# antonilo/unsupervised_detection

Measured on NVIDIA H100. Metric: frame-pairs/sec adversarial train step 256x448, higher is better.
Workload: dtype bf16

## Files before the change

### include/cis_b200.h

```cpp
#ifndef CIS_B200_H_
#define CIS_B200_H_
#include <stdint.h>
#include <stddef.h>

#ifdef __cplusplus
extern "C" {
#endif

typedef void* cis_stream_t;

enum { CIS_OK = 0, CIS_ERR_BAD_ARG = 1, CIS_ERR_UNSUPPORTED = 2, CIS_ERR_CUDA = 3 };
enum { CIS_ACT_NONE = 0, CIS_ACT_ELU = 1, CIS_ACT_LEAKY = 2 };
enum { CIS_MAX_TAPS = 49, CIS_MAX_SRC = 4 };

typedef struct {
  const void* ptr;
  int32_t pitch;
  int32_t c_off;
  int32_t chunks;
  int32_t n_mod;
} CisSrc;

typedef struct {
  int32_t N, H, W;
// ... 52 lines not shown
  int16_t dw[CIS_MAX_TAPS];
  int32_t nsrc;
  CisSrc src[CIS_MAX_SRC];
  const void* g;
  int32_t g_pitch, g_coff, g_chunks;
  float* dwp;
  int32_t Cout;
  int32_t K_pad;
  int32_t splits;
  int32_t tma;
  int32_t nh;
  int32_t nwg;
} CisWgrad;

const char* cis_last_error(void);
int cis_version(void);
uint32_t cis_crc32c(uint32_t crc, const void* data, size_t n);
int cis_host_resize_bilinear_legacy(const float* src, int32_t H, int32_t W, int32_t C, float* dst, int32_t OH, int32_t OW);
int cis_host_bgr8_to_rgb_resized(const unsigned char* bgr, int32_t H, int32_t W, float* dst, int32_t OH, int32_t OW);

int cis_conv_igemm(const CisConv* d, cis_stream_t stream);
int cis_conv_s2_phase_plan(const CisConv* d, CisConv* h, int16_t* wk);
int cis_set_persist_mode(int mode);
int cis_conv_wgrad(const CisWgrad* d, cis_stream_t stream);

int cis_pack_weights(const float* w, const int32_t* kmap, int32_t K_pad, int32_t rows, int32_t cout, int32_t sn, const int32_t* nmap,
                     void* wp, cis_stream_t stream);
int cis_pack_weights_tiled(const float* w, const int32_t* kmap, int32_t cin8, int32_t ntaps, int32_t n_tiles, int32_t BN, int32_t cout,
                           int32_t sn, const int32_t* nmap, void* out, int32_t thin, cis_stream_t stream);
int cis_unpack_wgrad(const float* dwp, const int32_t* kmap, int32_t K_pad, int32_t cout, int32_t nsplit, float* dw, const float* colpart,
                     int32_t nblocks, int32_t nch, float* db, int32_t layout, cis_stream_t stream);
int cis_bn_fold(const float* w, const float* bias, const float* gamma, const float* beta, int64_t nw, int32_t cout, float* w_eff,
                float* b_eff, cis_stream_t stream);
int cis_bn_chain(const float* w, const float* bias, const float* gamma, float* dw_eff_to_dw, const float* db_eff, int64_t nw,
                 int32_t cout, float* dbias, float* dgamma, float* dbeta, cis_stream_t stream);

enum { CIS_JOB_PACK = 0, CIS_JOB_PACK_TILED = 1, CIS_JOB_UNPACK = 2, CIS_JOB_BN_FOLD = 3, CIS_JOB_BN_CHAIN = 4 };
typedef struct {
  int32_t kind;
  int32_t i[8];
  int64_t n;
  const void* p[8];
} CisParamJob;
int cis_param_multi(const CisParamJob* jobs_dev, int32_t njobs, int32_t total_blocks, cis_stream_t stream);

int cis_dact_mul(void* g, int32_t g_pitch, int32_t g_coff, const void* y, int32_t y_pitch, int32_t y_coff, const void* res,
                 int32_t res_pitch, int32_t res_coff, int64_t npix, int32_t chunks, int32_t act, float alpha, cis_stream_t stream);
// ... 114 lines not shown
```

### unsupervised_detection_b200/_lib.py

```python
import ctypes as C
import os

_HERE = os.path.dirname(os.path.abspath(__file__))
LIB_PATH = os.path.join(_HERE, os.environ.get('CIS_LIB_NAME', 'libcis_b200.so'))

MAX_TAPS, MAX_SRC = 49, 4
ACT_NONE, ACT_ELU, ACT_LEAKY = 0, 1, 2
RESIZE_BILINEAR, RESIZE_NEAREST = 0, 1


class CisSrc(C.Structure):
    _fields_ = [('ptr', C.c_void_p), ('pitch', C.c_int32), ('c_off', C.c_int32), ('chunks', C.c_int32), ('n_mod', C.c_int32)]


class CisParamJob(C.Structure):
    _fields_ = [('kind', C.c_int32), ('i', C.c_int32 * 8), ('n', C.c_int64), ('p', C.c_void_p * 8)]


JOB_PACK, JOB_PACK_TILED, JOB_UNPACK, JOB_BN_FOLD, JOB_BN_CHAIN = range(5)


class CisSub(C.Structure):
    _fields_ = [('tap0', C.c_int32), ('ntaps', C.c_int32), ('hoy', C.c_int32), ('hox', C.c_int32), ('OH', C.c_int32), ('OW', C.c_int32),
                ('oa', C.c_int32), ('ob', C.c_int32), ('wpack', C.c_void_p)]
# ... 8 lines not shown
                ('bias', C.c_void_p), ('act', C.c_int32), ('alpha', C.c_float),
                ('DH', C.c_int32), ('DW', C.c_int32), ('osh', C.c_int32), ('osw', C.c_int32), ('oa', C.c_int32), ('ob', C.c_int32),
                ('out', C.c_void_p), ('out_pitch', C.c_int32), ('out_coff', C.c_int32), ('out_ch', C.c_int32),
                ('outf', C.c_void_p), ('outf_pitch', C.c_int32), ('outf_coff', C.c_int32), ('outf_ch', C.c_int32),
                ('add_pre', C.c_void_p), ('add_pre_pitch', C.c_int32), ('add_pre_coff', C.c_int32),
                ('addf_pre', C.c_void_p), ('addf_pitch', C.c_int32), ('addf_coff', C.c_int32),
                ('add_post', C.c_void_p), ('add_post_pitch', C.c_int32), ('add_post_coff', C.c_int32),
                ('mode', C.c_int32),
                ('halo', C.c_int32), ('dil', C.c_int32), ('MT', C.c_int32), ('hoy', C.c_int32), ('hox', C.c_int32),
                ('ey', C.c_int32), ('ex', C.c_int32),
                ('splits', C.c_int32), ('sk_scratch', C.c_void_p), ('sk_counters', C.c_void_p),
                ('nph', C.c_int32), ('ph_tap', C.c_int32 * 5), ('sk_cluster', C.c_int32),
                ('nsub', C.c_int32), ('sub', CisSub * 4), ('nwg', C.c_int32), ('thin', C.c_int32)]


class CisWgrad(C.Structure):
    _fields_ = [('N', C.c_int32), ('H', C.c_int32), ('W', C.c_int32), ('OH', C.c_int32), ('OW', C.c_int32),
                ('sh', C.c_int32), ('sw', C.c_int32), ('ntaps', C.c_int32),
                ('dh', C.c_int16 * MAX_TAPS), ('dw', C.c_int16 * MAX_TAPS),
                ('nsrc', C.c_int32), ('src', CisSrc * MAX_SRC),
                ('g', C.c_void_p), ('g_pitch', C.c_int32), ('g_coff', C.c_int32), ('g_chunks', C.c_int32),
                ('dwp', C.c_void_p), ('Cout', C.c_int32), ('K_pad', C.c_int32), ('splits', C.c_int32), ('tma', C.c_int32),
                ('nh', C.c_int32), ('nwg', C.c_int32)]


_i32, _i64, _f32, _p, _u64 = C.c_int32, C.c_int64, C.c_float, C.c_void_p, C.c_uint64

_PROTOS = {
    'cis_conv_igemm': [C.POINTER(CisConv)],
    'cis_conv_wgrad': [C.POINTER(CisWgrad)],
    'cis_pack_weights': [_p, _p, _i32, _i32, _i32, _i32, _p, _p],
    'cis_pack_weights_tiled': [_p, _p, _i32, _i32, _i32, _i32, _i32, _i32, _p, _p, _i32],
    'cis_unpack_wgrad': [_p, _p, _i32, _i32, _i32, _p, _p, _i32, _i32, _p, _i32],
    'cis_bn_fold': [_p, _p, _p, _p, _i64, _i32, _p, _p],
    'cis_param_multi': [_p, _i32, _i32],
    'cis_bn_chain': [_p, _p, _p, _p, _p, _i64, _i32, _p, _p, _p],
    'cis_dact_mul': [_p, _i32, _i32, _p, _i32, _i32, _p, _i32, _i32, _i64, _i32, _i32, _f32],
    'cis_add_slice': [_p, _i32, _i32, _p, _i32, _i32, _i64, _i32, _i32, _i32],
    'cis_colsum': [_p, _i32, _i32, _i64, _i32, _p, _i32],
    'cis_zero': [_p, _i64],
    'cis_dact_colsum': [_p, _i32, _i32, _p, _i32, _i32, _p, _i32, _i32, _i64, _i32, _i32, _f32, _p, _i32],
    'cis_resize_bilinear_bf16': [_p, _i32, _i32, _i32, _i32, _i32, _p, _i32, _i32, _i32, _i32, _i32],
    'cis_resize_concat_bf16': [C.POINTER(CisSrc), _i32, _i32, _i32, _i32, _p, _i32, _i32, _i32, _i32],
    'cis_resize_concat_bf16_bwd': [_p, _i32, _i32, _i32, _i32, _i32, C.POINTER(CisSrc), C.POINTER(C.c_int32), C.POINTER(C.c_int32), _i32, _i32, _i32],
    'cis_resize_bilinear_bf16_bwd': [_p, _i32, _i32, _i32, _i32, _i32, _p, _i32, _i32, _i32, _i32, _i32, _i32],
    'cis_resize_bilinear_f32': [_p, _i32, _i32, _i32, _i32, _p, _i32, _i32, _f32],
# ... 19 lines not shown
    'cis_cis_loss_reduce': [_p, _i32, _i32, _i64, _f32, _p, _p],
    'cis_cis_loss_bwd': [_p, _p, _p, _p, _p, _i32, _i32, _i32, _i32, _i32, _f32, _i32, _p, _p],
    'cis_resize_f32_bwd_to_bf16': [_p, _i32, _i32, _i32, _i32, _i32, _i32, _p, _i32],
    'cis_mask_bwd': [_p, _p, _p, _p, _i32, _i64, _p],
    'cis_abs_sum': [_p, _i64, _p],
    'cis_grad_avg_abs': [_p, _p, _i32, _p],
    'cis_clip_adam': [_p, _p, _p, _p, _i64, _f32, _f32, _f32, _f32, _f32, _f32, _p, _p, _i32, _u64],
    'cis_cast_f32_to_bf16': [_p, _i64, _p],
    'cis_cast_bf16_to_f32': [_p, _i64, _i32, _i32, _i32, _p],
    'cis_cast_bf16_to_f32_scaled': [_p, _i64, _i32, _i32, _i32, _f32, _p],
    'cis_charbonnier_bwd': [_p, _p, _p, _i32, _i64, _i32, _i32, _f32, _p, _p, _p, _p],
    'cis_dense_image_warp_bwd': [_p, _i32, _i32, _p, _f32, _i32, _i32, _i32, _i32, _p, _p, _p, _p],
    'cis_cost_volume_bwd': [_p, _i32, _i32, _p, _i32, _i32, _p, _i32, _i32, _i32, _i32, _p, _p, _p],
    'cis_resize_f32_bwd_to_bf16_scaled': [_p, _i32, _i32, _i32, _i32, _i32, _i32, _p, _i32, _f32],
    'cis_warp_costvol_bwd': [_p, _i32, _i32, _p, _i32, _i32, _p, _f32, _i32, _i32, _i32, _i32, _p, _i32, _i32, _p, _i32, _i32, _p, _i32, _i32,
                             _p, _i32, _i32, _i32, _p, _p, _p],
    'cis_parity_split_bf16': [_p, _i32, _i32, _i32, _i32, _i32, _i32, _p, _i32],
    'cis_warp_costvol_r': [_p, _i32, _i32, _p, _i32, _i32, _p, _f32, _i32, _i32, _i32, _i32, _p, _i32, _i32, _i32],
    'cis_cost_volume_bwd_r': [_p, _i32, _i32, _p, _i32, _i32, _p, _i32, _i32, _i32, _i32, _p, _p, _p, _i32],
    'cis_warp_costvol_bwd_r': [_p, _i32, _i32, _p, _i32, _i32, _p, _f32, _i32, _i32, _i32, _i32, _p, _i32, _i32, _p, _i32, _i32, _p, _i32, _i32,
                               _p, _i32, _i32, _i32, _p, _p, _p, _i32],
}
EXPORTS = sorted(list(_PROTOS) + ['cis_last_error', 'cis_version', 'cis_set_persist_mode', 'cis_crc32c', 'cis_host_resize_bilinear_legacy',
                                  'cis_host_bgr8_to_rgb_resized', 'cis_conv_s2_phase_plan'])

_lib = None


def load():
    global _lib
    if _lib is None:
        if not os.path.exists(LIB_PATH):
            raise RuntimeError('libcis_b200.so not built: run `python -c "import __graft_entry__ as g; g.build()"` '
                               '(no CPU fallback exists for the product path)')
        lib = C.CDLL(LIB_PATH)
        lib.cis_last_error.restype = C.c_char_p
        lib.cis_version.restype = C.c_int
        lib.cis_set_persist_mode.argtypes = [C.c_int]
        lib.cis_set_persist_mode.restype = C.c_int
        lib.cis_crc32c.argtypes = [C.c_uint32, C.c_void_p, C.c_size_t]
        lib.cis_crc32c.restype = C.c_uint32
        lib.cis_host_resize_bilinear_legacy.argtypes = [C.c_void_p, C.c_int32, C.c_int32, C.c_int32, C.c_void_p, C.c_int32, C.c_int32]
        lib.cis_host_resize_bilinear_legacy.restype = C.c_int
        lib.cis_host_bgr8_to_rgb_resized.argtypes = [C.c_void_p, C.c_int32, C.c_int32, C.c_void_p, C.c_int32, C.c_int32]
        lib.cis_host_bgr8_to_rgb_resized.restype = C.c_int
        lib.cis_conv_s2_phase_plan.argtypes = [C.POINTER(CisConv), C.POINTER(CisConv), C.POINTER(C.c_int16)]
        lib.cis_conv_s2_phase_plan.restype = C.c_int
        for name, args in _PROTOS.items():
            fn = getattr(lib, name)
            fn.argtypes = list(args) + [C.c_void_p]
            fn.restype = C.c_int
        _lib = lib
    return _lib


def check(rc, what=''):
    if rc != 0:
        raise RuntimeError('libcis_b200 %s failed (code %d): %s' % (what, rc, load().cis_last_error().decode()))


def call(name, *args):
    check(getattr(load(), name)(*args), name)
```

### unsupervised_detection_b200/csrc/conv_igemm.cu

```cuda
#include "ptx.cuh"
#include "../../include/cis_b200.h"
#include "common.cuh"
#include <cuda.h>
#include <stdlib.h>
#include <string.h>


namespace cis {

#ifdef CIS_TRACE
__device__ unsigned long long* g_trace = nullptr;
__device__ int g_trace_cap = 0;
#define CIS_TRACE_AT(slot)                                                                                         \
  do {                                                                                                             \
    if (g_trace && blockIdx.x == 0 && blockIdx.y == 0 && blockIdx.z == 0 && (slot) < g_trace_cap) g_trace[(slot)] = clock64(); \
  } while (0)
#else
#define CIS_TRACE_AT(slot) ((void)0)
#endif

static constexpr int kBM = 128;
static constexpr int kBK = 64;
static constexpr int kAStage = kBM * 128;
static constexpr int kThreads = 256;
// ... 1373 lines not shown
  static constexpr uint32_t kLayout = NH == 64 ? 1u : NH == 32 ? 2u : 3u;
};

template <int NH, int NWG>
__device__ __forceinline__ void wgrad_halo_wg_pairs(int w, int npairs, int cout, int& qa, int& np, int& hf) {
  constexpr int P = WgradHaloCfg<NH>::kPairs;
  const int nhalf = cout > 64 ? 2 : 1;
  if (NWG == 2 && nhalf == 2) {
    qa = blockIdx.z * P;
    np = min(P, npairs - qa);
    hf = w;
    return;
  }
  const int q0 = (blockIdx.z / nhalf) * (NWG * P);
  const int cnt = min(NWG * P, npairs - q0);
  const int h = NWG == 2 ? (cnt + 1) / 2 : cnt;
  qa = q0 + (w ? h : 0);
  np = w ? cnt - h : h;
  hf = blockIdx.z % nhalf;
}

template <int NH, int NWG>
__global__ void __launch_bounds__(128 * (1 + NWG)) conv_wgrad_halo_kernel(const __grid_constant__ CisWgrad p, const __grid_constant__ WgradHaloMaps maps,
                                                                          const int Wh, const int Hh, const int hoy, const int hox,
                                                                          const int stage_bytes, const int S) {
  using Cfg = WgradHaloCfg<NH>;
  constexpr int P = Cfg::kPairs;
  extern __shared__ uint8_t smem_raw[];
  __shared__ uint64_t bars[2 * kWHMaxStages + 1];
  __shared__ int s_off[CIS_MAX_TAPS + 1];
  const uint32_t tile_base = (smem_u32(smem_raw) + 1023u) & ~1023u;
  const uint32_t bar_full = smem_u32(&bars[0]);
  const uint32_t bar_empty = smem_u32(&bars[kWHMaxStages]);
  const uint32_t bar_accum = smem_u32(&bars[2 * kWHMaxStages]);
  const int tid = threadIdx.x, warp = tid >> 5, lane = tid & 31;
  pdl_launch_dependents();
  if (tid < p.ntaps) s_off[tid] = (p.dh[tid] - hoy) * Wh + (p.dw[tid] - hox);
  if (tid == p.ntaps) s_off[tid] = 0;
  const bool wg_halves = NWG == 2 && p.Cout > 64;
  const int ng = wg_halves ? 2 : 1;
  const int halo_bytes = stage_bytes - ng * (int)Cfg::kGTile;
  const int tiles_x = (p.OW + 7) / 8, tiles_y = (p.OH + 7) / 8;
  const int nkb_total = p.N * tiles_x * tiles_y;
  const int per = (nkb_total + (int)gridDim.y - 1) / (int)gridDim.y;
  const int kb0 = blockIdx.y * per;
  const int nkb = min(per, nkb_total - kb0);
  if (nkb <= 0) return;
  int m_chunks = 0;
  for (int i = 0; i < p.nsrc; ++i) m_chunks += p.src[i].chunks;
  const int nch64 = (m_chunks + 7) / 8;
  const int npairs = (p.ntaps + 1) / 2;
  const int c64 = blockIdx.x;

  if (tid == 128) {
    for (int s = 0; s < S; ++s) {
      mbar_init(bar_full + 8 * s, 1);
      mbar_init(bar_empty + 8 * s, NWG);
    }
    mbar_init(bar_accum, 128 * NWG);
    fence_mbar_init();
  }
// ... 1 lines not shown
  __syncthreads();

  if (warp < 4) {
    if (tid == 0) {
      int c = c64 * 8, si = 0;
      while (si < p.nsrc - 1 && c >= p.src[si].chunks) {
        c -= p.src[si].chunks;
        ++si;
      }
      int nm = p.src[0].n_mod;
      if (si == 1) nm = p.src[1].n_mod;
      if (si == 2) nm = p.src[2].n_mod;
      if (si == 3) nm = p.src[3].n_mod;
      int qa, np, hf0;
      wgrad_halo_wg_pairs<NH, NWG>(0, npairs, p.Cout, qa, np, hf0);
      const int tpi = tiles_x * tiles_y;
      for (int it = 0; it < nkb; ++it) {
        const int s = it % S;
        mbar_wait(bar_empty + 8 * s, (uint32_t)(((it / S) & 1) ^ 1));
        const int kb = kb0 + it;
        const int n = kb / tpi, r = kb - n * tpi;
        const int ty = r / tiles_x, tx = r - ty * tiles_x;
        const uint32_t st = tile_base + s * stage_bytes, bar = bar_full + 8 * s;
        mbar_expect_tx(bar, (uint32_t)(Wh * Hh * 128 + ng * (int)Cfg::kGTile));
        tma_load_4d(st, &maps.x[si], bar, c * 8, tx * 8 + hox, ty * 8 + hoy, nm ? (n % nm) : n);
        for (int h = 0; h < ng; ++h)
          tma_load_4d(st + halo_bytes + h * Cfg::kGTile, &maps.g, bar, (hf0 + h) * 64, tx * 8, ty * 8, n);
      }
    }
    __syncwarp();
    mbar_wait(bar_accum, 0);
    const int r = warp * 32 + lane;
    const int cch = r & 63;
    const uint32_t t_row = tile_base + (uint32_t)r * 16;
    for (int w = 0; w < NWG; ++w) {
      int qa, np, hf;
      wgrad_halo_wg_pairs<NH, NWG>(w, npairs, p.Cout, qa, np, hf);
      for (int q = 0; q < np; ++q) {
        const int t = 2 * (qa + q) + (r >> 6);
        if (t >= p.ntaps) continue;
        const size_t kcol = ((size_t)t * nch64 + c64) * 64 + cch;
#pragma unroll 1
        for (int c0 = 0; c0 < NH && hf * 64 + c0 < p.Cout; c0 += 16) {
          float v[16];
          acc_ld16(t_row + (uint32_t)((w * P + q) * NH + c0) * kAccColBytes, v);
          for (int e = 0; e < 16; ++e) {
            const int co = hf * 64 + c0 + e;
            if (co < p.Cout) p.dwp[((size_t)blockIdx.y * p.Cout + co) * p.K_pad + kcol] = v[e];
          }
        }
      }
    }
  } else {
    const int wg = NWG > 1 ? (warp - 4) >> 2 : 0;
    const int wtid = tid - 128 * (1 + wg);
    int qa, np, hf;
    wgrad_halo_wg_pairs<NH, NWG>(wg, npairs, p.Cout, qa, np, hf);
    np = __shfl_sync(0xffffffffu, np, 0);
    float acc[P][NH];
    const uint32_t ahi = desc_hi((uint32_t)(Wh * 128));
    const uint32_t bhi = (((8 * Cfg::kGRow) >> 4) & 0x3FFF) | (Cfg::kLayout << 30);
    const uint32_t kstep = (uint32_t)(2 * Wh * 128) >> 4;
    const uint32_t g_off = (uint32_t)halo_bytes + (wg_halves ? (uint32_t)wg * Cfg::kGTile : 0u);
    for (int it = 0; it < nkb; ++it) {
      const int s = it % S;
      mbar_wait(bar_full + 8 * s, (uint32_t)((it / S) & 1));
      const uint32_t st = tile_base + s * stage_bytes;
      const uint32_t blo0 = desc_lo(st + g_off, Cfg::kGTile);
      wg_fence();
#pragma unroll
      for (int q = 0; q < P; ++q) {
        if (q < np) {
          const int o0 = s_off[2 * (qa + q)], o1 = s_off[2 * (qa + q) + 1];
          const uint32_t lbo = (uint32_t)((o1 > o0 ? o1 - o0 : 1) * 128);
          const uint32_t alo0 = desc_lo(st + (uint32_t)(o0 * 128), lbo);
#pragma unroll
          for (int k = 0; k < 4; ++k)
            mma128<NH, 1, 1>(acc[q], alo0 + k * kstep, ahi, blo0 + Cfg::kGRow * k, bhi, lbo >> 4, (uint32_t)((it | k) != 0));
        }
      }
      wg_commit();
      wg_wait<0>();
      if (wtid == 0) mbar_arrive(bar_empty + 8 * s);
    }
    if constexpr (NWG > 1) asm volatile("bar.sync 1, %0;" ::"n"(128 * NWG) : "memory");
#pragma unroll
    for (int q = 0; q < P; ++q)
      if (q < np) acc_store<NH>(acc[q], tile_base + (uint32_t)((wg * P + q) * NH) * kAccColBytes, wtid);
    mbar_arrive(bar_accum);
  }
}

}

using namespace cis;

static bool pdl_enabled() {
  static const bool on = !(getenv("CIS_PDL") && atoi(getenv("CIS_PDL")) == 0);
  return on;
}
template <typename... KArgs, typename... Args>
static cudaError_t launch_pdl(void (*kern)(KArgs...), dim3 grid, dim3 block, size_t smem, cudaStream_t st, Args... args) {
  cudaLaunchConfig_t cfg;
  memset(&cfg, 0, sizeof(cfg));
  cfg.gridDim = grid;
  cfg.blockDim = block;
  cfg.dynamicSmemBytes = smem;
  cfg.stream = st;
  cudaLaunchAttribute attr[1];
  attr[0].id = cudaLaunchAttributeProgrammaticStreamSerialization;
  attr[0].val.programmaticStreamSerializationAllowed = 1;
// ... 377 lines not shown
      case 128: return d->nwg == 2 ? launch_halo<128, 2>(d, st) : launch_halo<128, 1>(d, st);
      default: return cis_set_error(CIS_ERR_UNSUPPORTED, "cis_conv_igemm: BN must be 16/32/64/128");
    }
  }
  CisConv h;
  int16_t wk[2 * CIS_MAX_TAPS];
  if (s2_phase_plan(d, &h, wk)) {
    switch (h.BN) {
      case 16: return launch_halo<16, 1>(&h, st, wk);
      case 32: return launch_halo<32, 1>(&h, st, wk);
      case 64: return launch_halo<64, 1>(&h, st, wk);
      case 128: return launch_halo<128, 1>(&h, st, wk);
    }
  }
  switch (d->BN) {
    case 16: return launch_fwd<16>(d, st);
    case 32: return launch_fwd<32>(d, st);
    case 64: return launch_fwd<64>(d, st);
    case 128: return launch_fwd<128>(d, st);
    default: return cis_set_error(CIS_ERR_UNSUPPORTED, "cis_conv_igemm: BN must be 16/32/64/128");
  }
}

template <int NH, int NWG>
static int launch_wgrad_halo_t(const CisWgrad* d, cudaStream_t st, int nch64, int Wh, int Hh, int hoy, int hox, int halo_bytes) {
  using Cfg = WgradHaloCfg<NH>;
  const bool wg_halves = NWG == 2 && d->Cout > 64;
  const int stage = halo_bytes + (wg_halves ? 2 : 1) * (int)Cfg::kGTile;
  const int npairs = (d->ntaps + 1) / 2, nhalf = d->Cout > 64 ? 2 : 1;
  const int gz = wg_halves ? (npairs + Cfg::kPairs - 1) / Cfg::kPairs : nhalf * ((npairs + NWG * Cfg::kPairs - 1) / (NWG * Cfg::kPairs));
  int S = (200 * 1024) / stage;
  if (S > kWHMaxStages) S = kWHMaxStages;
  if (S < 2) return cis_set_error(CIS_ERR_UNSUPPORTED, "cis_conv_wgrad(halo): halo does not fit shared memory");
  int smem = S * stage + 1024;
  const int acc_smem = NWG * kMaxAccCols * (int)kAccColBytes + 1024;
  if (smem < acc_smem) smem = acc_smem;
  static int attr_smem = 0;
  if (smem > attr_smem) {
    cudaError_t e = cudaFuncSetAttribute(conv_wgrad_halo_kernel<NH, NWG>, cudaFuncAttributeMaxDynamicSharedMemorySize, smem);
    if (e != cudaSuccess) return cis_set_cuda_error(e, "cudaFuncSetAttribute(conv_wgrad_halo)");
    attr_smem = smem;
  }
  WgradHaloMaps maps;
  memset(&maps, 0, sizeof(maps));
  CisSrc gs;
  gs.ptr = d->g; gs.pitch = d->g_pitch; gs.c_off = d->g_coff; gs.chunks = d->g_chunks; gs.n_mod = 0;
  const CUtensorMapSwizzle gswz = NH == 64 ? CU_TENSOR_MAP_SWIZZLE_128B : NH == 32 ? CU_TENSOR_MAP_SWIZZLE_64B : CU_TENSOR_MAP_SWIZZLE_32B;
  bool ok = encode_src_map(&maps.g, gs, d->N, d->OH, d->OW, 8, 8, 1, 0, 0, 1, NH, gswz);
  for (int i = 0; ok && i < d->nsrc; ++i) ok = encode_src_map(&maps.x[i], d->src[i], d->N, d->H, d->W, Wh, Hh);
  if (!ok) return cis_set_error(CIS_ERR_CUDA, "cis_conv_wgrad(halo): cuTensorMapEncodeTiled failed / unavailable");
  dim3 grid(nch64, d->splits, gz);
  cudaError_t le = launch_pdl(conv_wgrad_halo_kernel<NH, NWG>, grid, dim3(128 * (1 + NWG)), (size_t)smem, st, *d, maps, Wh, Hh, hoy, hox, stage, S);
  if (le != cudaSuccess) return cis_set_cuda_error(le, "launch(conv_wgrad_halo)");
  return cis_check_launch("conv_wgrad_halo");
}

static int launch_wgrad_halo(const CisWgrad* d, cudaStream_t st) {
  if (d->sh != 1 || d->sw != 1) return cis_set_error(CIS_ERR_BAD_ARG, "cis_conv_wgrad(halo): needs a stride-1 layer");
  int chunks = 0;
  for (int i = 0; i < d->nsrc; ++i) chunks += d->src[i].chunks;
  for (int i = 0; i < d->nsrc - 1; ++i)
    if (d->src[i].chunks % 8) return cis_set_error(CIS_ERR_BAD_ARG, "cis_conv_wgrad(halo): needs 64-channel aligned concat sources");
  const int nch64 = (chunks + 7) / 8;
  int hoy = d->dh[0], hox = d->dw[0], my = d->dh[0], mx = d->dw[0];
  for (int t = 1; t < d->ntaps; ++t) {
    if (d->dh[t] < hoy) hoy = d->dh[t];
    if (d->dw[t] < hox) hox = d->dw[t];
    if (d->dh[t] > my) my = d->dh[t];
    if (d->dw[t] > mx) mx = d->dw[t];
  }
  for (int t = 1; t < d->ntaps; ++t)
    if ((d->dh[t] - hoy) * 1024 + (d->dw[t] - hox) <= (d->dh[t - 1] - hoy) * 1024 + (d->dw[t - 1] - hox))
      return cis_set_error(CIS_ERR_BAD_ARG, "cis_conv_wgrad(halo): taps must be listed in increasing row-major order");
  const int Wh = 8 + (mx - hox), Hh = 8 + (my - hoy);
  if (Wh > 256 || Hh > 256) return cis_set_error(CIS_ERR_UNSUPPORTED, "cis_conv_wgrad(halo): tap extent too large");
  if (d->K_pad < d->ntaps * nch64 * 64) return cis_set_error(CIS_ERR_BAD_ARG, "cis_conv_wgrad(halo): K_pad smaller than taps * 64-channel groups");
  const int nh = d->nh ? d->nh : 64, nwg = d->nwg ? d->nwg : 1;
  if ((nh != 16 && nh != 32 && nh != 64) || nh < (d->Cout > 64 ? 64 : (d->Cout + 15) / 16 * 16) || nwg < 1 || nwg > 2)
    return cis_set_error(CIS_ERR_BAD_ARG, "cis_conv_wgrad(halo): nh must be 16/32/64 and cover Cout (64 above 64), nwg 1 or 2");
  const int halo_bytes = (Wh * Hh * 128 + 1023) & ~1023;
  switch (nh * 4 + nwg) {
    case 16 * 4 + 1: return launch_wgrad_halo_t<16, 1>(d, st, nch64, Wh, Hh, hoy, hox, halo_bytes);
    case 16 * 4 + 2: return launch_wgrad_halo_t<16, 2>(d, st, nch64, Wh, Hh, hoy, hox, halo_bytes);
    case 32 * 4 + 1: return launch_wgrad_halo_t<32, 1>(d, st, nch64, Wh, Hh, hoy, hox, halo_bytes);
    case 32 * 4 + 2: return launch_wgrad_halo_t<32, 2>(d, st, nch64, Wh, Hh, hoy, hox, halo_bytes);
    case 64 * 4 + 1: return launch_wgrad_halo_t<64, 1>(d, st, nch64, Wh, Hh, hoy, hox, halo_bytes);
    default: return launch_wgrad_halo_t<64, 2>(d, st, nch64, Wh, Hh, hoy, hox, halo_bytes);
  }
}

extern "C" int cis_conv_wgrad(const CisWgrad* d, cis_stream_t stream) {
  if (!d || d->ntaps < 1 || d->ntaps > CIS_MAX_TAPS || d->nsrc < 1 || d->nsrc > CIS_MAX_SRC || d->K_pad % 64 != 0 || d->Cout < 1 ||
      d->Cout > 128 || d->splits < 1 || !d->g || !d->dwp)
    return cis_set_error(CIS_ERR_BAD_ARG, "cis_conv_wgrad: bad descriptor");
  {
    const long M = (long)d->N * d->OH * d->OW;
    const long nkb_total = d->tma ? (long)d->N * ((d->OW + 7) / 8) * ((d->OH + 7) / 8) : (M + 63) / 64;
    const long per = (nkb_total + d->splits - 1) / d->splits;
    if ((long)(d->splits - 1) * per >= nkb_total) return cis_set_error(CIS_ERR_BAD_ARG, "cis_conv_wgrad: a split would own no reduction block");
  }
  if (d->tma == 2) return launch_wgrad_halo(d, (cudaStream_t)stream);
  static bool attr_set = false;
  if (!attr_set) {
    cudaError_t e = cudaFuncSetAttribute(conv_wgrad_kernel, cudaFuncAttributeMaxDynamicSharedMemorySize, kWSmem);
    if (e != cudaSuccess) return cis_set_cuda_error(e, "cudaFuncSetAttribute(conv_wgrad)");
    attr_set = true;
  }
  WgradMaps maps;
  memset(&maps, 0, sizeof(maps));
  if (d->tma) {
    if (d->sh != 1 || d->sw != 1) return cis_set_error(CIS_ERR_BAD_ARG, "cis_conv_wgrad: TMA path needs a stride-1 layer");
    for (int i = 0; i < d->nsrc - 1; ++i)
      if (d->src[i].chunks % 8) return cis_set_error(CIS_ERR_BAD_ARG, "cis_conv_wgrad: TMA path needs 64-channel aligned concat sources");
    CisSrc gs;
    gs.ptr = d->g; gs.pitch = d->g_pitch; gs.c_off = d->g_coff; gs.chunks = d->g_chunks; gs.n_mod = 0;
    bool ok = encode_src_map(&maps.g, gs, d->N, d->OH, d->OW, 8, 8);
    for (int i = 0; ok && i < d->nsrc; ++i) ok = encode_src_map(&maps.x[i], d->src[i], d->N, d->H, d->W, 8, 8);
    if (!ok) return cis_set_error(CIS_ERR_CUDA, "cis_conv_wgrad: cuTensorMapEncodeTiled failed / unavailable");
  }
  dim3 grid((d->K_pad + 127) / 128, d->splits);
  cudaError_t le = launch_pdl(conv_wgrad_kernel, grid, dim3(d->tma ? kThreads : kGThreads), kWSmem, (cudaStream_t)stream, *d, maps);
  if (le != cudaSuccess) return cis_set_cuda_error(le, "launch(conv_wgrad)");
  return cis_check_launch("conv_wgrad");
}
// ... 1 lines not shown
```

### unsupervised_detection_b200/engine.py

```python
import ctypes as C
import dataclasses
import os

import numpy as np
import torch

from . import _lib
from ._lib import CisConv, CisWgrad, CisSrc, ACT_NONE, ACT_ELU, ACT_LEAKY


def ru(x, m):
    return (x + m - 1) // m * m


def same_pad(n_in, k, s=1, d=1):
    out = -(-n_in // s)
    total = max((out - 1) * s + (k - 1) * d + 1 - n_in, 0)
    return total // 2, total - total // 2


SIDE_STREAM = True
_SIDE = {}
MULTI_PARAM_OPS = os.environ.get('CIS_MULTI_PARAM', '1') == '1'
DACT_COLSUM = os.environ.get('CIS_DACT_COLSUM', '1') == '1'
# ... 258 lines not shown
WGRAD_TMA = True
MATERIALIZE_MISALIGNED_CONCAT = True


WGRAD_CTAS_PER_SM = int(os.environ.get('CIS_WGRAD_CTAS_PER_SM', '2'))
WGRAD_MAX_SLICE_MB = float(os.environ.get('CIS_WGRAD_MAX_SLICE_MB', '16'))
WGRAD_HALO_MIN_CH = int(os.environ.get('CIS_WGRAD_HALO_MIN_CH', '16'))
WGRAD_HALO = os.environ.get('CIS_WGRAD_HALO', '1') == '1'


def wgrad_halo_fits(taps, cout, stride):
    if stride != 1 or not taps:
        return False
    hoy, hox = min(a for a, _ in taps), min(b for _, b in taps)
    keys = [(a - hoy) * 1024 + (b - hox) for a, b in taps]
    if any(k1 <= k0 for k0, k1 in zip(keys, keys[1:])):
        return False
    wh, hh = 8 + max(b for _, b in taps) - hox, 8 + max(a for a, _ in taps) - hoy
    nh = 64 if cout > 64 else ru(cout, 16)
    if ((len(taps) + 1) // 2) * nh > 512 or wh > 256 or hh > 256:
        return False
    stage = ru(wh * hh * 128, 1024) + 8192 * (2 if WGRAD_HALO_NWG >= 2 and cout > 64 else 1)
    return (200 * 1024) // stage >= 2


WGRAD_HALO_NWG = int(os.environ.get('CIS_WGRAD_HALO_NWG', '2'))


def wgrad_splits(nkb, ntile, cout, K_pad):
    splits = max(1, min(nkb // 8 if nkb >= 8 else 1, max(1, (WGRAD_CTAS_PER_SM * NUM_SMS) // ntile)))
    if WGRAD_MAX_SLICE_MB > 0:
        splits = max(1, min(splits, int(WGRAD_MAX_SLICE_MB * 1e6 / (cout * K_pad * 4.0))))
    return -(-nkb // (-(-nkb // splits)))


def wgrad_halo_tiling(ntaps, cout):
    npairs = (ntaps + 1) // 2
    if WGRAD_HALO_NWG < 2:
        return 64, 1, (2 if cout > 64 else 1) * (-(-npairs // 2))
    nh = 64 if cout > 64 else ru(cout, 16)
    p = MAX_ACC_COLS // nh
    if cout > 64:
        return 64, 2, -(-npairs // p)
    nwg = 2 if npairs > p else 1
    return nh, nwg, -(-npairs // (nwg * p))

# ... 870 lines not shown
```

Measured before the change: 662.7.

## Route stride-1/2 wgrad through phase-split halo TMA kernel with thin-channel variant

Non-TMA weight-gradient convolutions that fit now go through a host plan that splits stride-2 layers into four phase planes. Each phase is loaded as a halo tile by TMA, so a stride-2 layer runs as a stride-1 one in the halo wgmma kernel. A new thin kernel serves single-chunk inputs with Cout up to 32 by packing taps into shared-memory blocks, and it writes results in an interleaved layout. This aims to replace the generic wgrad path with higher input reuse, at the cost of more complex planning, a new output layout, and new bounds conditions.

```diff
diff --git a/include/cis_b200.h b/include/cis_b200.h
--- a/include/cis_b200.h
+++ b/include/cis_b200.h
@@ -98,7 +98,23 @@
 int cis_conv_igemm(const CisConv* d, cis_stream_t stream);
 int cis_conv_s2_phase_plan(const CisConv* d, CisConv* h, int16_t* wk);
 int cis_set_persist_mode(int mode);
+#define CIS_WGRAD_MAX_BLK 14
+typedef struct {
+  int32_t nph;
+  int32_t ph_tap[5];
+  int32_t Wh, Hh, hoy, hox;
+  int32_t plane_bytes;
+  int32_t stage_bytes, stages;
+  int32_t grid[3];
+  int32_t layout;
+  int16_t tap[CIS_MAX_TAPS];
+  int16_t off[CIS_MAX_TAPS + 1];
+  int32_t compact, nblk;
+  int32_t blk_off[CIS_WGRAD_MAX_BLK];
+  int16_t blk_tap[CIS_WGRAD_MAX_BLK][8];
+} CisWgradHaloPlan;
 int cis_conv_wgrad(const CisWgrad* d, cis_stream_t stream);
+int cis_conv_wgrad_halo_plan(const CisWgrad* d, CisWgrad* h, CisWgradHaloPlan* pl);
 
 int cis_pack_weights(const float* w, const int32_t* kmap, int32_t K_pad, int32_t rows, int32_t cout, int32_t sn, const int32_t* nmap,
                      void* wp, cis_stream_t stream);
diff --git a/unsupervised_detection_b200/_lib.py b/unsupervised_detection_b200/_lib.py
--- a/unsupervised_detection_b200/_lib.py
+++ b/unsupervised_detection_b200/_lib.py
@@ -54,6 +54,13 @@
                 ('g', C.c_void_p), ('g_pitch', C.c_int32), ('g_coff', C.c_int32), ('g_chunks', C.c_int32),
                 ('dwp', C.c_void_p), ('Cout', C.c_int32), ('K_pad', C.c_int32), ('splits', C.c_int32), ('tma', C.c_int32),
                 ('nh', C.c_int32), ('nwg', C.c_int32)]
+
+
+class CisWgradHaloPlan(C.Structure):
+    _fields_ = [('nph', C.c_int32), ('ph_tap', C.c_int32 * 5), ('Wh', C.c_int32), ('Hh', C.c_int32), ('hoy', C.c_int32), ('hox', C.c_int32),
+                ('plane_bytes', C.c_int32), ('stage_bytes', C.c_int32), ('stages', C.c_int32), ('grid', C.c_int32 * 3), ('layout', C.c_int32),
+                ('tap', C.c_int16 * MAX_TAPS), ('off', C.c_int16 * (MAX_TAPS + 1)), ('compact', C.c_int32), ('nblk', C.c_int32),
+                ('blk_off', C.c_int32 * 14), ('blk_tap', (C.c_int16 * 8) * 14)]
 
 
 _i32, _i64, _f32, _p, _u64 = C.c_int32, C.c_int64, C.c_float, C.c_void_p, C.c_uint64
@@ -119,7 +126,7 @@
                                _p, _i32, _i32, _i32, _p, _p, _p, _i32],
 }
 EXPORTS = sorted(list(_PROTOS) + ['cis_last_error', 'cis_version', 'cis_set_persist_mode', 'cis_crc32c', 'cis_host_resize_bilinear_legacy',
-                                  'cis_host_bgr8_to_rgb_resized', 'cis_conv_s2_phase_plan'])
+                                  'cis_host_bgr8_to_rgb_resized', 'cis_conv_s2_phase_plan', 'cis_conv_wgrad_halo_plan'])
 
 _lib = None
 
@@ -143,6 +150,8 @@
         lib.cis_host_bgr8_to_rgb_resized.restype = C.c_int
         lib.cis_conv_s2_phase_plan.argtypes = [C.POINTER(CisConv), C.POINTER(CisConv), C.POINTER(C.c_int16)]
         lib.cis_conv_s2_phase_plan.restype = C.c_int
+        lib.cis_conv_wgrad_halo_plan.argtypes = [C.POINTER(CisWgrad), C.POINTER(CisWgrad), C.POINTER(CisWgradHaloPlan)]
+        lib.cis_conv_wgrad_halo_plan.restype = C.c_int
         for name, args in _PROTOS.items():
             fn = getattr(lib, name)
             fn.argtypes = list(args) + [C.c_void_p]
diff --git a/unsupervised_detection_b200/csrc/conv_igemm.cu b/unsupervised_detection_b200/csrc/conv_igemm.cu
--- a/unsupervised_detection_b200/csrc/conv_igemm.cu
+++ b/unsupervised_detection_b200/csrc/conv_igemm.cu
@@ -1419,21 +1419,22 @@
 
 template <int NH, int NWG>
 __global__ void __launch_bounds__(128 * (1 + NWG)) conv_wgrad_halo_kernel(const __grid_constant__ CisWgrad p, const __grid_constant__ WgradHaloMaps maps,
-                                                                          const int Wh, const int Hh, const int hoy, const int hox,
-                                                                          const int stage_bytes, const int S) {
+                                                                          const __grid_constant__ CisWgradHaloPlan pl) {
   using Cfg = WgradHaloCfg<NH>;
+  const int Wh = pl.Wh, Hh = pl.Hh, hoy = pl.hoy, hox = pl.hox, stage_bytes = pl.stage_bytes, S = pl.stages;
   constexpr int P = Cfg::kPairs;
   extern __shared__ uint8_t smem_raw[];
   __shared__ uint64_t bars[2 * kWHMaxStages + 1];
   __shared__ int s_off[CIS_MAX_TAPS + 1];
+  __shared__ int s_tap[CIS_MAX_TAPS];
   const uint32_t tile_base = (smem_u32(smem_raw) + 1023u) & ~1023u;
   const uint32_t bar_full = smem_u32(&bars[0]);
   const uint32_t bar_empty = smem_u32(&bars[kWHMaxStages]);
   const uint32_t bar_accum = smem_u32(&bars[2 * kWHMaxStages]);
   const int tid = threadIdx.x, warp = tid >> 5, lane = tid & 31;
   pdl_launch_dependents();
-  if (tid < p.ntaps) s_off[tid] = (p.dh[tid] - hoy) * Wh + (p.dw[tid] - hox);
-  if (tid == p.ntaps) s_off[tid] = 0;
+  if (tid <= p.ntaps) s_off[tid] = pl.off[tid];
+  if (tid < p.ntaps) s_tap[tid] = pl.tap[tid];
   const bool wg_halves = NWG == 2 && p.Cout > 64;
   const int ng = wg_halves ? 2 : 1;
   const int halo_bytes = stage_bytes - ng * (int)Cfg::kGTile;
@@ -1481,8 +1482,13 @@
         const int n = kb / tpi, r = kb - n * tpi;
         const int ty = r / tiles_x, tx = r - ty * tiles_x;
         const uint32_t st = tile_base + s * stage_bytes, bar = bar_full + 8 * s;
-        mbar_expect_tx(bar, (uint32_t)(Wh * Hh * 128 + ng * (int)Cfg::kGTile));
-        tma_load_4d(st, &maps.x[si], bar, c * 8, tx * 8 + hox, ty * 8 + hoy, nm ? (n % nm) : n);
+        mbar_expect_tx(bar, (uint32_t)(pl.nph * Wh * Hh * 128 + ng * (int)Cfg::kGTile));
+        if (pl.nph == 1) {
+          tma_load_4d(st, &maps.x[si], bar, c * 8, tx * 8 + hox, ty * 8 + hoy, nm ? (n % nm) : n);
+        } else {
+          for (int q = 0; q < 4; ++q)
+            tma_load_4d(st + q * pl.plane_bytes, &maps.x[q], bar, c * 8, tx * 8 + hox, ty * 8 + hoy, nm ? (n % nm) : n);
+        }
         for (int h = 0; h < ng; ++h)
           tma_load_4d(st + halo_bytes + h * Cfg::kGTile, &maps.g, bar, (hf0 + h) * 64, tx * 8, ty * 8, n);
       }
@@ -1498,14 +1504,17 @@
       for (int q = 0; q < np; ++q) {
         const int t = 2 * (qa + q) + (r >> 6);
         if (t >= p.ntaps) continue;
-        const size_t kcol = ((size_t)t * nch64 + c64) * 64 + cch;
+        if (pl.layout && c64 * 64 + cch >= m_chunks * 8) continue;
+        const size_t kcol = pl.layout ? (size_t)s_tap[t] * (m_chunks * 8) + c64 * 64 + cch : ((size_t)t * nch64 + c64) * 64 + cch;
+        float* const o = p.dwp + (size_t)blockIdx.y * p.Cout * p.K_pad + (pl.layout ? (kcol >> 2) * p.Cout * 4 + (kcol & 3) : kcol);
+        const size_t so = pl.layout ? 4 : (size_t)p.K_pad;
 #pragma unroll 1
         for (int c0 = 0; c0 < NH && hf * 64 + c0 < p.Cout; c0 += 16) {
           float v[16];
           acc_ld16(t_row + (uint32_t)((w * P + q) * NH + c0) * kAccColBytes, v);
           for (int e = 0; e < 16; ++e) {
             const int co = hf * 64 + c0 + e;
-            if (co < p.Cout) p.dwp[((size_t)blockIdx.y * p.Cout + co) * p.K_pad + kcol] = v[e];
+            if (co < p.Cout) o[co * so] = v[e];
           }
         }
       }
@@ -1546,6 +1555,114 @@
 #pragma unroll
     for (int q = 0; q < P; ++q)
       if (q < np) acc_store<NH>(acc[q], tile_base + (uint32_t)((wg * P + q) * NH) * kAccColBytes, wtid);
+    mbar_arrive(bar_accum);
+  }
+}
+
+
+template <int NH, int NB>
+__global__ void __launch_bounds__(256) conv_wgrad_thin_kernel(const __grid_constant__ CisWgrad p, const __grid_constant__ WgradHaloMaps maps,
+                                                              const __grid_constant__ CisWgradHaloPlan pl) {
+  using Cfg = WgradHaloCfg<NH>;
+  extern __shared__ uint8_t smem_raw[];
+  __shared__ uint64_t bars[2 * kWHMaxStages + 1];
+  const uint32_t tile_base = (smem_u32(smem_raw) + 1023u) & ~1023u;
+  const uint32_t bar_full = smem_u32(&bars[0]);
+  const uint32_t bar_empty = smem_u32(&bars[kWHMaxStages]);
+  const uint32_t bar_accum = smem_u32(&bars[2 * kWHMaxStages]);
+  const int tid = threadIdx.x, warp = tid >> 5;
+  pdl_launch_dependents();
+  const int Wh = pl.Wh, Hh = pl.Hh, S = pl.stages, stage_bytes = pl.stage_bytes;
+  const uint32_t g_off = (uint32_t)stage_bytes - Cfg::kGTile;
+  const int tiles_x = (p.OW + 7) / 8, tiles_y = (p.OH + 7) / 8;
+  const int nkb_total = p.N * tiles_x * tiles_y;
+  const int per = (nkb_total + (int)gridDim.y - 1) / (int)gridDim.y;
+  const int kb0 = blockIdx.y * per;
+  const int nkb = min(per, nkb_total - kb0);
+  if (nkb <= 0) return;
+  constexpr uint32_t kBlkBytes = (NH / 4) * 1024;
+  if (tid == 128) {
+    for (int s = 0; s < S; ++s) {
+      mbar_init(bar_full + 8 * s, 1);
+      mbar_init(bar_empty + 8 * s, 1);
+    }
+    mbar_init(bar_accum, 128);
+    fence_mbar_init();
+  }
+  pdl_wait();
+  __syncthreads();
+
+  if (warp < 4) {
+    if (tid == 0) {
+      const int nm = p.src[0].n_mod, tpi = tiles_x * tiles_y;
+      for (int it = 0; it < nkb; ++it) {
+        const int s = it % S;
+        mbar_wait(bar_empty + 8 * s, (uint32_t)(((it / S) & 1) ^ 1));
+        const int kb = kb0 + it;
+        const int n = kb / tpi, r = kb - n * tpi;
+        const int ty = r / tiles_x, tx = r - ty * tiles_x;
+        const uint32_t st = tile_base + s * stage_bytes, bar = bar_full + 8 * s;
+        mbar_expect_tx(bar, (uint32_t)(pl.nph * Wh * Hh * 16) + Cfg::kGTile);
+        for (int q = 0; q < pl.nph; ++q)
+          tma_load_4d(st + q * pl.plane_bytes, &maps.x[q], bar, 0, tx * 8 + pl.hox, ty * 8 + pl.hoy, nm ? (n % nm) : n);
+        tma_load_4d(st + g_off, &maps.g, bar, 0, tx * 8, ty * 8, n);
+      }
+    }
+    __syncwarp();
+    mbar_wait(bar_accum, 0);
+    float* const slice = p.dwp + (size_t)blockIdx.y * p.Cout * p.K_pad;
+    for (int i = tid; i < pl.nblk * 64; i += 128) {
+      const int b = i >> 6, r = i & 63;
+      const int t = pl.blk_tap[b][r >> 3];
+      if (t < 0) continue;
+      const int kcol = t * 8 + (r & 7);
+      float* const o = slice + (size_t)(kcol >> 2) * p.Cout * 4 + (kcol & 3);
+      const uint32_t a = tile_base + (uint32_t)b * kBlkBytes + (uint32_t)r * 16;
+      for (int co = 0; co < p.Cout; ++co) {
+        float v;
+        asm volatile("ld.shared.f32 %0, [%1];" : "=f"(v) : "r"(a + (uint32_t)(co >> 2) * 1024 + (uint32_t)(co & 3) * 4) : "memory");
+        o[co * 4] = v;
+      }
+    }
+  } else {
+    const int wtid = tid - 128;
+    float acc[NB][NH / 2];
+    const uint32_t ahi = desc_hi_ns(16);
+    const uint32_t bhi = (((8 * Cfg::kGRow) >> 4) & 0x3FFF) | (Cfg::kLayout << 30);
+    const uint32_t kstep = (uint32_t)(2 * Wh);
+    for (int it = 0; it < nkb; ++it) {
+      const int s = it % S;
+      mbar_wait(bar_full + 8 * s, (uint32_t)((it / S) & 1));
+      const uint32_t st = tile_base + s * stage_bytes;
+      const uint32_t blo0 = desc_lo(st + g_off, Cfg::kGTile);
+      wg_fence();
+#pragma unroll
+      for (int b = 0; b < NB; ++b) {
+        if (b < pl.nblk) {
+          const uint32_t alo0 = desc_lo(st + (uint32_t)pl.blk_off[b] * 16, (uint32_t)Wh * 16);
+#pragma unroll
+          for (int k = 0; k < 4; ++k)
+            Wgmma<NH, 1, 1>::mma(acc[b], ((uint64_t)ahi << 32) | (alo0 + k * kstep), ((uint64_t)bhi << 32) | (blo0 + Cfg::kGRow * k),
+                                 (uint32_t)((it | k) != 0));
+        }
+      }
+      wg_commit();
+      wg_wait<0>();
+      if (wtid == 0) mbar_arrive(bar_empty + 8 * s);
+    }
+    const int w = wtid >> 5, lane = wtid & 31;
+#pragma unroll
+    for (int b = 0; b < NB; ++b) {
+      if (b < pl.nblk) {
+#pragma unroll
+        for (int i = 0; i < NH / 8; ++i) {
+          const int col = 8 * i + 2 * (lane & 3);
+          const uint32_t a = tile_base + (uint32_t)b * kBlkBytes + (uint32_t)((col >> 2) * 1024 + (16 * w + (lane >> 2)) * 16 + (col & 3) * 4);
+          asm volatile("st.shared.v2.f32 [%0], {%1, %2};" ::"r"(a), "f"(acc[b][4 * i]), "f"(acc[b][4 * i + 1]) : "memory");
+          asm volatile("st.shared.v2.f32 [%0], {%1, %2};" ::"r"(a + 8 * 16), "f"(acc[b][4 * i + 2]), "f"(acc[b][4 * i + 3]) : "memory");
+        }
+      }
+    }
     mbar_arrive(bar_accum);
   }
 }
@@ -1969,17 +2086,40 @@
   }
 }
 
+static bool wgrad_halo_geometry(const CisWgrad* h, CisWgradHaloPlan* pl) {
+  int chunks = 0;
+  for (int i = 0; i < h->nsrc; ++i) chunks += h->src[i].chunks;
+  int hoy = h->dh[0], hox = h->dw[0], my = h->dh[0], mx = h->dw[0];
+  for (int t = 1; t < h->ntaps; ++t) {
+    hoy = min(hoy, (int)h->dh[t]);
+    hox = min(hox, (int)h->dw[t]);
+    my = max(my, (int)h->dh[t]);
+    mx = max(mx, (int)h->dw[t]);
+  }
+  const int Wh = 8 + (mx - hox), Hh = 8 + (my - hoy);
+  if (Wh > 256 || Hh > 256) return false;
+  const int nh = h->nh ? h->nh : 64, nwg = h->nwg ? h->nwg : 1;
+  const int P = kMaxAccCols / nh, npairs = (h->ntaps + 1) / 2, nhalf = h->Cout > 64 ? 2 : 1;
+  const bool wg_halves = nwg == 2 && h->Cout > 64;
+  pl->Wh = Wh; pl->Hh = Hh; pl->hoy = hoy; pl->hox = hox;
+  pl->plane_bytes = (Wh * Hh * 128 + 1023) & ~1023;
+  pl->stage_bytes = pl->nph * pl->plane_bytes + (wg_halves ? 2 : 1) * 64 * 2 * nh;
+  pl->stages = min((200 * 1024) / pl->stage_bytes, kWHMaxStages);
+  if (pl->stages < 2) return false;
+  pl->grid[0] = (chunks + 7) / 8;
+  pl->grid[1] = h->splits;
+  pl->grid[2] = wg_halves ? (npairs + P - 1) / P : nhalf * ((npairs + nwg * P - 1) / (nwg * P));
+  for (int q = 0; q < pl->nph; ++q)
+    for (int t = pl->ph_tap[q]; t < pl->ph_tap[q + 1]; ++t)
+      pl->off[t] = (int16_t)(q * (pl->plane_bytes / 128) + (h->dh[t] - hoy) * Wh + (h->dw[t] - hox));
+  pl->off[h->ntaps] = 0;
+  return true;
+}
+
 template <int NH, int NWG>
-static int launch_wgrad_halo_t(const CisWgrad* d, cudaStream_t st, int nch64, int Wh, int Hh, int hoy, int hox, int halo_bytes) {
+static int launch_wgrad_halo_t(const CisWgrad* d, cudaStream_t st, const CisWgradHaloPlan& pl) {
   using Cfg = WgradHaloCfg<NH>;
-  const bool wg_halves = NWG == 2 && d->Cout > 64;
-  const int stage = halo_bytes + (wg_halves ? 2 : 1) * (int)Cfg::kGTile;
-  const int npairs = (d->ntaps + 1) / 2, nhalf = d->Cout > 64 ? 2 : 1;
-  const int gz = wg_halves ? (npairs + Cfg::kPairs - 1) / Cfg::kPairs : nhalf * ((npairs + NWG * Cfg::kPairs - 1) / (NWG * Cfg::kPairs));
-  int S = (200 * 1024) / stage;
-  if (S > kWHMaxStages) S = kWHMaxStages;
-  if (S < 2) return cis_set_error(CIS_ERR_UNSUPPORTED, "cis_conv_wgrad(halo): halo does not fit shared memory");
-  int smem = S * stage + 1024;
+  int smem = pl.stages * pl.stage_bytes + 1024;
   const int acc_smem = NWG * kMaxAccCols * (int)kAccColBytes + 1024;
   if (smem < acc_smem) smem = acc_smem;
   static int attr_smem = 0;
@@ -1994,12 +2134,27 @@
   gs.ptr = d->g; gs.pitch = d->g_pitch; gs.c_off = d->g_coff; gs.chunks = d->g_chunks; gs.n_mod = 0;
   const CUtensorMapSwizzle gswz = NH == 64 ? CU_TENSOR_MAP_SWIZZLE_128B : NH == 32 ? CU_TENSOR_MAP_SWIZZLE_64B : CU_TENSOR_MAP_SWIZZLE_32B;
   bool ok = encode_src_map(&maps.g, gs, d->N, d->OH, d->OW, 8, 8, 1, 0, 0, 1, NH, gswz);
-  for (int i = 0; ok && i < d->nsrc; ++i) ok = encode_src_map(&maps.x[i], d->src[i], d->N, d->H, d->W, Wh, Hh);
+  if (pl.nph == 1) {
+    for (int i = 0; ok && i < d->nsrc; ++i) ok = encode_src_map(&maps.x[i], d->src[i], d->N, d->H, d->W, pl.Wh, pl.Hh);
+  } else {
+    for (int q = 0; ok && q < 4; ++q) ok = encode_src_map(&maps.x[q], d->src[0], d->N, d->H, d->W, pl.Wh, pl.Hh, 2, q >> 1, q & 1);
+  }
   if (!ok) return cis_set_error(CIS_ERR_CUDA, "cis_conv_wgrad(halo): cuTensorMapEncodeTiled failed / unavailable");
-  dim3 grid(nch64, d->splits, gz);
-  cudaError_t le = launch_pdl(conv_wgrad_halo_kernel<NH, NWG>, grid, dim3(128 * (1 + NWG)), (size_t)smem, st, *d, maps, Wh, Hh, hoy, hox, stage, S);
+  dim3 grid(pl.grid[0], pl.grid[1], pl.grid[2]);
+  cudaError_t le = launch_pdl(conv_wgrad_halo_kernel<NH, NWG>, grid, dim3(128 * (1 + NWG)), (size_t)smem, st, *d, maps, pl);
   if (le != cudaSuccess) return cis_set_cuda_error(le, "launch(conv_wgrad_halo)");
   return cis_check_launch("conv_wgrad_halo");
+}
+
+static int launch_wgrad_halo_nh(const CisWgrad* d, cudaStream_t st, const CisWgradHaloPlan& pl) {
+  switch ((d->nh ? d->nh : 64) * 4 + (d->nwg ? d->nwg : 1)) {
+    case 16 * 4 + 1: return launch_wgrad_halo_t<16, 1>(d, st, pl);
+    case 16 * 4 + 2: return launch_wgrad_halo_t<16, 2>(d, st, pl);
+    case 32 * 4 + 1: return launch_wgrad_halo_t<32, 1>(d, st, pl);
+    case 32 * 4 + 2: return launch_wgrad_halo_t<32, 2>(d, st, pl);
+    case 64 * 4 + 1: return launch_wgrad_halo_t<64, 1>(d, st, pl);
+    default: return launch_wgrad_halo_t<64, 2>(d, st, pl);
+  }
 }
 
 static int launch_wgrad_halo(const CisWgrad* d, cudaStream_t st) {
@@ -2009,31 +2164,128 @@
   for (int i = 0; i < d->nsrc - 1; ++i)
     if (d->src[i].chunks % 8) return cis_set_error(CIS_ERR_BAD_ARG, "cis_conv_wgrad(halo): needs 64-channel aligned concat sources");
   const int nch64 = (chunks + 7) / 8;
-  int hoy = d->dh[0], hox = d->dw[0], my = d->dh[0], mx = d->dw[0];
-  for (int t = 1; t < d->ntaps; ++t) {
-    if (d->dh[t] < hoy) hoy = d->dh[t];
-    if (d->dw[t] < hox) hox = d->dw[t];
-    if (d->dh[t] > my) my = d->dh[t];
-    if (d->dw[t] > mx) mx = d->dw[t];
-  }
   for (int t = 1; t < d->ntaps; ++t)
-    if ((d->dh[t] - hoy) * 1024 + (d->dw[t] - hox) <= (d->dh[t - 1] - hoy) * 1024 + (d->dw[t - 1] - hox))
+    if (d->dh[t] * 1024 + d->dw[t] <= d->dh[t - 1] * 1024 + d->dw[t - 1])
       return cis_set_error(CIS_ERR_BAD_ARG, "cis_conv_wgrad(halo): taps must be listed in increasing row-major order");
-  const int Wh = 8 + (mx - hox), Hh = 8 + (my - hoy);
-  if (Wh > 256 || Hh > 256) return cis_set_error(CIS_ERR_UNSUPPORTED, "cis_conv_wgrad(halo): tap extent too large");
   if (d->K_pad < d->ntaps * nch64 * 64) return cis_set_error(CIS_ERR_BAD_ARG, "cis_conv_wgrad(halo): K_pad smaller than taps * 64-channel groups");
   const int nh = d->nh ? d->nh : 64, nwg = d->nwg ? d->nwg : 1;
   if ((nh != 16 && nh != 32 && nh != 64) || nh < (d->Cout > 64 ? 64 : (d->Cout + 15) / 16 * 16) || nwg < 1 || nwg > 2)
     return cis_set_error(CIS_ERR_BAD_ARG, "cis_conv_wgrad(halo): nh must be 16/32/64 and cover Cout (64 above 64), nwg 1 or 2");
-  const int halo_bytes = (Wh * Hh * 128 + 1023) & ~1023;
-  switch (nh * 4 + nwg) {
-    case 16 * 4 + 1: return launch_wgrad_halo_t<16, 1>(d, st, nch64, Wh, Hh, hoy, hox, halo_bytes);
-    case 16 * 4 + 2: return launch_wgrad_halo_t<16, 2>(d, st, nch64, Wh, Hh, hoy, hox, halo_bytes);
-    case 32 * 4 + 1: return launch_wgrad_halo_t<32, 1>(d, st, nch64, Wh, Hh, hoy, hox, halo_bytes);
-    case 32 * 4 + 2: return launch_wgrad_halo_t<32, 2>(d, st, nch64, Wh, Hh, hoy, hox, halo_bytes);
-    case 64 * 4 + 1: return launch_wgrad_halo_t<64, 1>(d, st, nch64, Wh, Hh, hoy, hox, halo_bytes);
-    default: return launch_wgrad_halo_t<64, 2>(d, st, nch64, Wh, Hh, hoy, hox, halo_bytes);
-  }
+  CisWgradHaloPlan pl;
+  memset(&pl, 0, sizeof(pl));
+  pl.nph = 1;
+  for (int q = 1; q < 5; ++q) pl.ph_tap[q] = d->ntaps;
+  for (int t = 0; t < d->ntaps; ++t) pl.tap[t] = (int16_t)t;
+  if (!wgrad_halo_geometry(d, &pl)) return cis_set_error(CIS_ERR_UNSUPPORTED, "cis_conv_wgrad(halo): tap extent too large or halo does not fit shared memory");
+  return launch_wgrad_halo_nh(d, st, pl);
+}
+
+static bool wgrad_thin_plan(const CisWgrad* g, CisWgrad* h, CisWgradHaloPlan* pl) {
+  if (g->nsrc != 1 || g->src[0].chunks != 1 || g->Cout > 32) return false;
+  const int nt = h->ntaps, nh = g->Cout > 16 ? 32 : 16;
+  int hoy = h->dh[0], hox = h->dw[0], my = h->dh[0], mx = h->dw[0];
+  for (int t = 1; t < nt; ++t) {
+    hoy = min(hoy, (int)h->dh[t]);
+    hox = min(hox, (int)h->dw[t]);
+    my = max(my, (int)h->dh[t]);
+    mx = max(mx, (int)h->dw[t]);
+  }
+  const int Wh = 8 + (mx - hox), Hh = 8 + (my - hoy);
+  if (Wh > 256 || Hh > 256) return false;
+  const int plane = (Wh * Hh * 16 + 127) & ~127;
+  int nblk = 0;
+  for (int q = 0; q < pl->nph; ++q)
+    for (int t = pl->ph_tap[q]; t < pl->ph_tap[q + 1]; ++t) {
+      const bool open = t == pl->ph_tap[q] || h->dh[t] != h->dh[t - 1] ||
+                        (plane / 16) * q + (h->dh[t] - hoy) * Wh + (h->dw[t] - hox) - pl->blk_off[nblk - 1] > 7;
+      if (open) {
+        if (nblk == CIS_WGRAD_MAX_BLK) return false;
+        pl->blk_off[nblk] = (plane / 16) * q + (h->dh[t] - hoy) * Wh + (h->dw[t] - hox);
+        for (int j = 0; j < 8; ++j) pl->blk_tap[nblk][j] = -1;
+        ++nblk;
+      }
+      pl->blk_tap[nblk - 1][(plane / 16) * q + (h->dh[t] - hoy) * Wh + (h->dw[t] - hox) - pl->blk_off[nblk - 1]] = pl->tap[t];
+    }
+  if (nblk * nh / 2 > 112) return false;
+  pl->nblk = nblk;
+  pl->Wh = Wh; pl->Hh = Hh; pl->hoy = hoy; pl->hox = hox;
+  pl->plane_bytes = plane;
+  pl->stage_bytes = ((pl->nph * plane + 256 + 1023) & ~1023) + 64 * 2 * nh;
+  pl->stages = min((200 * 1024) / pl->stage_bytes, kWHMaxStages);
+  pl->grid[0] = 1; pl->grid[1] = g->splits; pl->grid[2] = 1;
+  h->nh = nh;
+  h->nwg = 1;
+  const long nkb = (long)g->N * ((g->OW + 7) / 8) * ((g->OH + 7) / 8), per = (nkb + g->splits - 1) / g->splits;
+  pl->compact = pl->stages >= 2 && nkb >= 296 && (long)(g->splits - 1) * per < nkb;
+  return pl->compact != 0;
+}
+
+template <int NH, int NB>
+static int launch_wgrad_thin_t(const CisWgrad* d, cudaStream_t st, const CisWgradHaloPlan& pl) {
+  int smem = pl.stages * pl.stage_bytes + 1024;
+  const int acc_smem = pl.nblk * (NH / 4) * 1024 + 1024;
+  if (smem < acc_smem) smem = acc_smem;
+  static int attr_smem = 0;
+  if (smem > attr_smem) {
+    cudaError_t e = cudaFuncSetAttribute(conv_wgrad_thin_kernel<NH, NB>, cudaFuncAttributeMaxDynamicSharedMemorySize, smem);
+    if (e != cudaSuccess) return cis_set_cuda_error(e, "cudaFuncSetAttribute(conv_wgrad_thin)");
+    attr_smem = smem;
+  }
+  WgradHaloMaps maps;
+  memset(&maps, 0, sizeof(maps));
+  CisSrc gs;
+  gs.ptr = d->g; gs.pitch = d->g_pitch; gs.c_off = d->g_coff; gs.chunks = d->g_chunks; gs.n_mod = 0;
+  bool ok = encode_src_map(&maps.g, gs, d->N, d->OH, d->OW, 8, 8, 1, 0, 0, 1, NH, NH == 32 ? CU_TENSOR_MAP_SWIZZLE_64B : CU_TENSOR_MAP_SWIZZLE_32B);
+  for (int q = 0; ok && q < pl.nph; ++q)
+    ok = encode_src_map(&maps.x[q], d->src[0], d->N, d->H, d->W, pl.Wh, pl.Hh, pl.nph == 4 ? 2 : 1, q >> 1, q & 1, 1, 8, CU_TENSOR_MAP_SWIZZLE_NONE);
+  if (!ok) return cis_set_error(CIS_ERR_CUDA, "cis_conv_wgrad(thin): cuTensorMapEncodeTiled failed / unavailable");
+  cudaError_t le = launch_pdl(conv_wgrad_thin_kernel<NH, NB>, dim3(1, pl.grid[1], 1), dim3(256), (size_t)smem, st, *d, maps, pl);
+  if (le != cudaSuccess) return cis_set_cuda_error(le, "launch(conv_wgrad_thin)");
+  return cis_check_launch("conv_wgrad_thin");
+}
+
+static bool wgrad_phase_plan(const CisWgrad* g, CisWgrad* h, CisWgradHaloPlan* pl) {
+  const char* sw = getenv("CIS_WGRAD_PHASE");
+  if ((sw && atoi(sw) == 0) || g->tma != 0 || g->sh != g->sw || (g->sh != 1 && g->sh != 2) || (g->sh == 2 && (g->nsrc != 1 || g->H < 2 || g->W < 2)))
+    return false;
+  int chunks = 0;
+  for (int i = 0; i < g->nsrc; ++i) {
+    chunks += g->src[i].chunks;
+    if ((i < g->nsrc - 1 && g->src[i].chunks % 8) || (g->src[i].pitch | g->src[i].c_off) % 8 ||
+        ((uintptr_t)g->src[i].ptr + (size_t)g->src[i].c_off * 2) % 16)
+      return false;
+  }
+  const int nt = g->ntaps, sft = g->sh - 1;
+  if (g->K_pad < nt * chunks * 8 || ((uintptr_t)g->g + (size_t)g->g_coff * 2) % 16 || (g->g_pitch | g->g_coff) % 8) return false;
+  *h = *g;
+  memset(pl, 0, sizeof(*pl));
+  pl->nph = sft ? 4 : 1;
+  pl->layout = 1;
+  int k = 0;
+  for (int q = 0; q < 4; ++q) {
+    for (int t = 0; t < nt; ++t)
+      if ((sft ? ((g->dh[t] & 1) << 1 | (g->dw[t] & 1)) : 0) == q) {
+        h->dh[k] = (int16_t)(g->dh[t] >> sft);
+        h->dw[k] = (int16_t)(g->dw[t] >> sft);
+        if (k > pl->ph_tap[q] && h->dh[k] * 1024 + h->dw[k] <= h->dh[k - 1] * 1024 + h->dw[k - 1]) return false;
+        pl->tap[k++] = (int16_t)t;
+      }
+    pl->ph_tap[q + 1] = k;
+  }
+  h->sh = h->sw = 1;
+  h->tma = 2;
+  if (wgrad_thin_plan(g, h, pl)) return true;
+  const int npairs = (nt + 1) / 2;
+  h->nh = g->Cout > 64 ? 64 : (g->Cout + 15) / 16 * 16;
+  h->nwg = g->Cout > 64 || npairs > kMaxAccCols / h->nh ? 2 : 1;
+  if (!wgrad_halo_geometry(h, pl) || pl->grid[2] > 4) return false;
+  const long nkb = (long)g->N * ((g->OW + 7) / 8) * ((g->OH + 7) / 8), per = (nkb + g->splits - 1) / g->splits;
+  return nkb >= 296 && (long)(g->splits - 1) * per < nkb;
+}
+extern "C" int cis_conv_wgrad_halo_plan(const CisWgrad* d, CisWgrad* h, CisWgradHaloPlan* pl) {
+  return d && h && pl && d->ntaps >= 1 && d->ntaps <= CIS_MAX_TAPS && d->nsrc >= 1 && d->nsrc <= CIS_MAX_SRC && d->Cout >= 1 && d->Cout <= 128 &&
+                 d->splits >= 1 && wgrad_phase_plan(d, h, pl)
+             ? 1 : 0;
 }
 
 extern "C" int cis_conv_wgrad(const CisWgrad* d, cis_stream_t stream) {
@@ -2047,6 +2299,14 @@
     if ((long)(d->splits - 1) * per >= nkb_total) return cis_set_error(CIS_ERR_BAD_ARG, "cis_conv_wgrad: a split would own no reduction block");
   }
   if (d->tma == 2) return launch_wgrad_halo(d, (cudaStream_t)stream);
+  {
+    CisWgrad h;
+    CisWgradHaloPlan pl;
+    if (wgrad_phase_plan(d, &h, &pl)) {
+      if (!pl.compact) return launch_wgrad_halo_nh(&h, (cudaStream_t)stream, pl);
+      return h.nh == 32 ? launch_wgrad_thin_t<32, 7>(&h, (cudaStream_t)stream, pl) : launch_wgrad_thin_t<16, 14>(&h, (cudaStream_t)stream, pl);
+    }
+  }
   static bool attr_set = false;
   if (!attr_set) {
     cudaError_t e = cudaFuncSetAttribute(conv_wgrad_kernel, cudaFuncAttributeMaxDynamicSharedMemorySize, kWSmem);
diff --git a/unsupervised_detection_b200/engine.py b/unsupervised_detection_b200/engine.py
--- a/unsupervised_detection_b200/engine.py
+++ b/unsupervised_detection_b200/engine.py
@@ -304,6 +304,11 @@
         return False
     stage = ru(wh * hh * 128, 1024) + 8192 * (2 if WGRAD_HALO_NWG >= 2 and cout > 64 else 1)
     return (200 * 1024) // stage >= 2
+
+
+def wgrad_halo_rewrite(d):
+    h, pl = CisWgrad(), _lib.CisWgradHaloPlan()
+    return (h, pl) if _lib.load().cis_conv_wgrad_halo_plan(C.byref(d), C.byref(h), C.byref(pl)) else None
 
 
 WGRAD_HALO_NWG = int(os.environ.get('CIS_WGRAD_HALO_NWG', '2'))
```

Result: faster. 681.3, median of 6 (+2.8%).
